# JohnLonginotto/uq

Measured on NVIDIA B200. Metric: fastq_to_uq_encode_reads_per_s, higher is better.
Workload: dtype u8

## Files before the change

### uq_b200/csrc/hist_units.cuh

```cuda
#pragma once
#include "tile.cuh"

#define H2_THREADS 1024
#define H2_QLO 33u
#define H2_ROWS 95
#define H2_COLS 512
#define H2_NOHINT 0x00060402u

struct h2_core {
    unsigned hist_b[256];
    unsigned hist_q[H2_ROWS + 1];
    int state[256];
    unsigned hints, dirty, oor, qmax;
};

__device__ __forceinline__ uint4 lds_v4(uint32_t a) {
    uint4 v;
    asm volatile("ld.shared.v4.u32 {%0, %1, %2, %3}, [%4];" : "=r"(v.x), "=r"(v.y), "=r"(v.z), "=r"(v.w) : "r"(a));
    return v;
}
__device__ __forceinline__ uint32_t h2_unitmask(int lo, int hi) {
    const uint32_t l = lo < 0 ? 0u : (uint32_t)lo, h = hi > 16 ? 16u : (uint32_t)hi;
    return h > l ? (((1u << h) - 1u) & ~((1u << l) - 1u)) : 0u;
}
__device__ __forceinline__ uint32_t h2_nibble_bytes(uint32_t nib) {
    return (((nib & 15u) * 0x00204081u) & 0x01010101u) * 0xFFu;
}

__device__ __forceinline__ unsigned h2_bytesum(unsigned x) {
    const unsigned y = (x & 0x00FF00FFu) + ((x >> 8) & 0x00FF00FFu);
    return (y & 0xFFFFu) + (y >> 16);
}

__device__ __forceinline__ void h2_slow_byte(h2_core* S, unsigned b, unsigned q) {
    atomicAdd(&S->hist_b[b], 1u);
    int f = S->state[b];
    if (f != (int)q && f != 256) {
        if (f < 0) {
            const int old = atomicCAS(&S->state[b], -1, (int)q);
            if (old >= 0 && old != (int)q) { S->state[b] = 256; S->dirty = 1u; }
        } else {
            S->state[b] = 256; S->dirty = 1u;
        }
    }
}

struct h2_dna_acc {
    unsigned p0, p1, p01;
    unsigned ocnt;
    unsigned words, zeroed, noff;
};

__device__ __noinline__ void h2_dna_flush_vals(h2_core* S, unsigned p0, unsigned p1, unsigned p01, unsigned ocnt, unsigned words,
                                               unsigned zeroed, unsigned H) {
    const unsigned s0 = h2_bytesum(p0), s1 = h2_bytesum(p1) >> 1, s01 = h2_bytesum(p01);
    const unsigned n3 = s01, n1 = s0 - s01, n2 = s1 - s01, n0 = 4u * words - zeroed - n1 - n2 - n3;
    const unsigned v0 = n0 - (ocnt & 255u), v1 = n1 - ((ocnt >> 8) & 255u), v2 = n2 - ((ocnt >> 16) & 255u), v3 = n3 - (ocnt >> 24);
    if (v0) atomicAdd(&S->hist_b[H & 255u], v0);
    if (v1) atomicAdd(&S->hist_b[(H >> 8) & 255u], v1);
    if (v2) atomicAdd(&S->hist_b[(H >> 16) & 255u], v2);
    if (v3) atomicAdd(&S->hist_b[H >> 24], v3);
}
__device__ __forceinline__ void h2_dna_flush(h2_core* S, h2_dna_acc& A, unsigned H) {
    h2_dna_flush_vals(S, A.p0, A.p1, A.p01, A.ocnt, A.words, A.zeroed, H);
    A.p0 = A.p1 = A.p01 = A.ocnt = A.words = A.zeroed = A.noff = 0;
}

__device__ __forceinline__ void h2_dna_flush_warp(h2_core* S, h2_dna_acc& A, unsigned H, unsigned lane) {
    unsigned s0 = h2_bytesum(A.p0), s1 = h2_bytesum(A.p1) >> 1, s01 = h2_bytesum(A.p01);
    unsigned nw = A.words, nz = A.zeroed;
    unsigned oc[4];
#pragma unroll
    for (unsigned c = 0; c < 4; c++) oc[c] = (A.ocnt >> (8 * c)) & 255u;
    s0 = __reduce_add_sync(0xffffffffu, s0); s1 = __reduce_add_sync(0xffffffffu, s1); s01 = __reduce_add_sync(0xffffffffu, s01);
    nw = __reduce_add_sync(0xffffffffu, nw); nz = __reduce_add_sync(0xffffffffu, nz);
#pragma unroll
    for (unsigned c = 0; c < 4; c++) oc[c] = __reduce_add_sync(0xffffffffu, oc[c]);
    if (lane == 0 && nw) {
        unsigned n[4];
        n[3] = s01; n[1] = s0 - s01; n[2] = s1 - s01;
        n[0] = 4u * nw - nz - n[1] - n[2] - n[3];
#pragma unroll
        for (unsigned c = 0; c < 4; c++) {
            const unsigned v = n[c] - oc[c];
            if (v) atomicAdd(&S->hist_b[(H >> (8 * c)) & 255u], v);
        }
    }
    A.p0 = A.p1 = A.p01 = A.ocnt = A.words = A.zeroed = A.noff = 0;
}

__device__ __forceinline__ void h2_dna_unit(h2_core* S, const uint4 v, uint32_t ua, uint32_t delta, int lo, int hi, unsigned H,
                                            h2_dna_acc& A) {
    unsigned w[4] = {v.x, v.y, v.z, v.w}, t[4], bad[4];
#pragma unroll
    for (int k = 0; k < 4; k++) {
        t[k] = (w[k] >> 1) & 0x03030303u;
        const unsigned u2 = t[k] | (t[k] >> 4);
        const unsigned sel = __byte_perm(u2, 0u, 0x4420);
        unsigned ex;
        asm("prmt.b32 %0, %1, %2, %3;" : "=r"(ex) : "r"(H), "r"(0u), "r"(sel));
        bad[k] = ex ^ w[k];
    }
    if (lo > 0 || hi < 16) {
        const uint32_t vb = h2_unitmask(lo, hi);
#pragma unroll
        for (int k = 0; k < 4; k++) {
            const unsigned vm = h2_nibble_bytes(vb >> (4 * k));
            bad[k] &= vm;
            t[k] &= vm;
        }
        A.zeroed += 16u - __popc(vb);
    }
    if (bad[0] | bad[1] | bad[2] | bad[3]) {
        unsigned m = 0;
#pragma unroll
        for (int k = 0; k < 4; k++) {
            const unsigned z = (((bad[k] & 0x7F7F7F7Fu) + 0x7F7F7F7Fu) | bad[k]) & 0x80808080u;
            m |= z >> (7 - k);
        }
        A.noff += __popc(m);
        do {
            const unsigned i = (unsigned)__ffs((int)m) - 1u;
            m &= m - 1u;
            const unsigned pos = 4u * (i & 7u) + (i >> 3);
            const unsigned b = lds_u8(ua + pos), q = lds_u8(ua + pos + delta);
            A.ocnt += 1u << (8u * ((b >> 1) & 3u));
            h2_slow_byte(S, b, q);
        } while (m);
    }
#pragma unroll
    for (int k = 0; k < 4; k++) {
        A.p0 += t[k] & 0x01010101u;
        A.p1 += t[k] & 0x02020202u;
        A.p01 += t[k] & (t[k] >> 1) & 0x01010101u;
    }
    A.words += 4u;
}

__device__ __forceinline__ bool h2_qual_unit(const uint4 v, int lo, int hi, uint32_t qcol) {
    unsigned w[4] = {v.x, v.y, v.z, v.w};
    unsigned bad = 0;
    if (lo > 0 || hi < 16) {
        const uint32_t vb = h2_unitmask(lo, hi);
#pragma unroll
        for (int k = 0; k < 4; k++) {
            const unsigned vm = h2_nibble_bytes(vb >> (4 * k));
            const unsigned chk = (w[k] & vm) | (0x21212121u & ~vm);
            bad |= ((chk | (chk + 0x01010101u)) | ~((chk & 0x7F7F7F7Fu) + 0x5F5F5F5Fu)) & 0x80808080u;
            w[k] = (w[k] & vm) | (0x7F7F7F7Fu & ~vm);
        }
    } else {
#pragma unroll
        for (int k = 0; k < 4; k++)
            bad |= ((w[k] | (w[k] + 0x01010101u)) | ~((w[k] & 0x7F7F7F7Fu) + 0x5F5F5F5Fu)) & 0x80808080u;
    }
    if (bad) return false;
#pragma unroll
    for (int k = 0; k < 4; k++) {
#pragma unroll
        for (int j = 0; j < 4; j++) {
            const uint32_t a = qcol + (__byte_perm(w[k], 0u, 0x4440 | j) << 9);
            sts_u8(a, lds_u8m(a) + 1u);
        }
    }
    return true;
}

__device__ __noinline__ void h2_qual_flush(h2_core* S, uint32_t qcol) {
    for (unsigned r = 0; r < H2_ROWS; r++) {
        const uint32_t a = qcol + ((r + H2_QLO) << 9);
        const unsigned c = lds_u8m(a);
        if (c) { atomicAdd(&S->hist_q[r], c); sts_u8(a, 0u); }
    }
}

#define H3_STAGES 3
struct h3_smem {
    alignas(128) uint8_t front_pad[128];
    alignas(128) uint8_t bytes[H3_STAGES][TL_CAP + 32];
    uint32_t loff[H3_STAGES][4 * TL_R + 4];
    alignas(8) uint64_t full[H3_STAGES];
    alignas(8) uint64_t empty[H3_STAGES];
    uint32_t ok[H3_STAGES];
    alignas(16) uint8_t qcnt[H2_ROWS * H2_COLS];
    h2_core C;
};

__device__ __forceinline__ void mbar_arrive(uint64_t* bar) {
    asm volatile("mbarrier.arrive.shared::cta.b64 _, [%0];" ::"r"(smem_u32(bar)) : "memory");
}

__global__ void __launch_bounds__(H2_THREADS, 1) k_pair_hist_pipe(const uint8_t* __restrict__ d, uint64_t n_bytes,
                                                                 const uint64_t* __restrict__ line_off, uint64_t r_begin, uint64_t n_reads,
                                                                 an_dev* __restrict__ s, unsigned int* __restrict__ fallback,
                                                                 uint8_t* __restrict__ names, uint32_t name_pitch) {
    static_assert(TL_R == 128, "thread <-> line binding assumes 128 records per tile");
    extern __shared__ __align__(128) uint8_t h3_raw[];
    h3_smem* S = reinterpret_cast<h3_smem*>(h3_raw);
    const unsigned tid = threadIdx.x, lane = tid & 31u, wid = tid >> 5;
    for (unsigned i = tid; i < H2_ROWS * H2_COLS / 4; i += H2_THREADS) reinterpret_cast<uint32_t*>(S->qcnt)[i] = 0;
    for (unsigned i = tid; i <= H2_ROWS; i += H2_THREADS) S->C.hist_q[i] = 0;
    if (tid < 256) { S->C.hist_b[tid] = 0; S->C.state[tid] = -1; }
    if (tid == 0) {
        S->C.hints = H2_NOHINT; S->C.dirty = 0; S->C.oor = 0; S->C.qmax = 0;
        for (int st = 0; st < H3_STAGES; st++) { mbar_init(&S->full[st], H2_THREADS / 32); mbar_init(&S->empty[st], H2_THREADS / 32); }
        asm volatile("fence.mbarrier_init.release.cluster;" ::: "memory");
    }
    __syncthreads();
    const unsigned line = tid & 255u, rec = line & 127u, k0 = tid >> 8;
    const bool isq = (line >> 7) != 0;
    const bool producer = wid == H2_THREADS / 32 - 1;
    const unsigned cw = ((wid >> 3) << 2) | (wid & 3u);
    const uint32_t qcol = smem_u32(S->qcnt) + lane * 4u + (cw & 3u) + 128u * (cw >> 2) - (H2_QLO << 9);
    unsigned qsym = 0;
    h2_dna_acc A;
    A.p0 = A.p1 = A.p01 = A.ocnt = A.words = A.zeroed = A.noff = 0;
    unsigned H = H2_NOHINT;
    unsigned long long len_min = ~0ull, len_max = 0ull;
    long long bad_plus = LLONG_MAX, bad_len = LLONG_MAX;

    const uint64_t ntiles = (n_reads - r_begin + TL_R - 1) / TL_R;
    const uint32_t K = blockIdx.x < ntiles ? (uint32_t)((ntiles - blockIdx.x + gridDim.x - 1) / gridDim.x) : 0u;

    constexpr uint32_t OPW = (4 * TL_R + 1 + H2_THREADS / 32 - 1) / (H2_THREADS / 32);
    uint64_t pend_off = 0, pend_b0 = 0, pend_b1 = 0;
    const uint64_t rstride = (uint64_t)gridDim.x * TL_R;
    const uint32_t my_off = wid * OPW + lane;
    auto nrec_at = [&](uint64_t r0) { return (uint32_t)(n_reads - r0 < TL_R ? n_reads - r0 : TL_R); };
    auto prep_load = [&](uint64_t r0, uint32_t nrec) {
        const uint64_t* lo = line_off + 4 * r0;
        if (lane < OPW && my_off <= 4 * nrec) pend_off = __ldg(lo + my_off);
        if (producer && lane == 0) { pend_b0 = __ldg(lo); pend_b1 = __ldg(lo + 4 * nrec); }
    };
    auto prep_store = [&](uint32_t nrec, uint32_t st, bool wait_empty, uint32_t empty_par) {
        if (wait_empty) mbar_wait(&S->empty[st], empty_par);
        const uint32_t i = my_off;
        if (lane < OPW && i <= 4 * nrec) S->loff[st][i] = (uint32_t)pend_off;
        if (producer) {
            const uint64_t b0 = __shfl_sync(0xffffffffu, pend_b0, 0), b1 = __shfl_sync(0xffffffffu, pend_b1, 0);
            const uint64_t a0 = b0 & ~15ull;
            const bool fits = b1 - a0 <= TL_CAP;
            uint64_t a1 = (b1 + 15) & ~15ull;
            const uint64_t lim = n_bytes & ~15ull;
            if (a1 > lim) a1 = lim;
            if (a1 < a0) a1 = a0;
            if (fits) for (uint64_t q = a1 + lane; q < b1; q += 32) S->bytes[st][q - a0] = d[q];
            __syncwarp();
            if (lane == 0) {
                S->ok[st] = fits ? 1u : 0u;
                const uint32_t bulk = fits ? (uint32_t)(a1 - a0) : 0u;
                asm volatile("fence.proxy.async.shared::cta;" ::: "memory");
                mbar_expect_tx(&S->full[st], bulk);
                if (bulk) bulk_g2s(S->bytes[st], d + a0, bulk, &S->full[st]);
            }
        } else {
            __syncwarp();
            if (lane == 0) mbar_arrive(&S->full[st]);
        }
    };

    {
        uint64_t r0p = r_begin + (uint64_t)blockIdx.x * TL_R;
        for (uint32_t k = 0; k < K && k < H3_STAGES - 1; k++, r0p += rstride) { const uint32_t nr = nrec_at(r0p); prep_load(r0p, nr); prep_store(nr, k, false, 0u); }
    }
    uint32_t F = 1, next_flush = 1;
    uint64_t r0 = r_begin + (uint64_t)blockIdx.x * TL_R;
    uint32_t st = 0, par = 0;
    for (uint32_t k = 0; k < K; k++) {
        const bool ahead = k + H3_STAGES - 1 < K;
        const uint64_t r0a = r0 + 2 * rstride;
        const uint32_t nrec_a = ahead ? nrec_at(r0a) : 0u;
        const uint32_t st_a = st ? st - 1u : 2u;
        const uint32_t par_a = st ? par : par ^ 1u;
        if (ahead) prep_load(r0a, nrec_a);
        mbar_wait(&S->full[st], par);
        const uint32_t nrec = nrec_at(r0);
        if (S->ok[st] && names && wid < TL_R / 8) {
            const uint32_t bytes_a = smem_u32(S->bytes[st]);
            const uint32_t* loff = S->loff[st];
            const uint32_t base32 = loff[0] & ~15u;
            const uint32_t nr = 8u * wid + (lane >> 2);
            if (nr < nrec) {
                const uint32_t n0 = loff[4 * nr] - base32, nlen = loff[4 * nr + 1] - base32 - n0 - 1u;
                if (nlen + 1u > name_pitch || nlen > 255u) {
                    if ((lane & 3u) == 0) atomicOr(&S->C.oor, 2u);
                } else {
                    uint4* dst = reinterpret_cast<uint4*>(names + (r0 + nr) * name_pitch);
                    for (uint32_t c = lane & 3u; 16u * c <= nlen; c += 4) {
                        const uint32_t at = n0 + 16u * c - 1u, al = bytes_a + (at & ~3u), sh = (at & 3u) * 8u;
                        const uint32_t x0 = lds_u32(al), x1 = lds_u32(al + 4u), x2 = lds_u32(al + 8u), x3 = lds_u32(al + 12u), x4 = lds_u32(al + 16u);
                        uint4 v;
                        v.x = __funnelshift_r(x0, x1, sh); v.y = __funnelshift_r(x1, x2, sh);
                        v.z = __funnelshift_r(x2, x3, sh); v.w = __funnelshift_r(x3, x4, sh);
                        if (c == 0) v.x = (v.x & 0xFFFFFF00u) | nlen;
                        dst[c] = v;
                    }
                }
            }
        }
        if (!S->ok[st]) {
            if (tid == 0) atomicOr(fallback, 1u);
        } else if (rec < nrec) {
            const uint32_t bytes_a = smem_u32(S->bytes[st]);
            const uint32_t* loff = S->loff[st];
            const uint32_t base32 = loff[0] & ~15u;
            const uint32_t o1 = loff[4 * rec + 1] - base32, o2 = loff[4 * rec + 2] - base32, o3 = loff[4 * rec + 3] - base32,
                           o4 = loff[4 * rec + 4] - base32;
            uint32_t len = o2 - o1 - 1;
            const uint32_t qlen = o4 - o3 - 1;
            if (tid < TL_R) {
                const long long r = (long long)(r0 + rec);
                if (len != qlen && r < bad_len) bad_len = r;
                len_min = len < len_min ? len : len_min; len_max = len > len_max ? len : len_max;
                const unsigned plus = o3 - o2 < 2u ? 0u : lds_u8(bytes_a + o2);
                if (plus != '+' && r < bad_plus) bad_plus = r;
            }
            if (qlen < len) len = qlen;
            const uint32_t sb = isq ? o3 : o1, eb = sb + len;
            for (uint32_t u = (sb & ~15u) + 16u * k0; u < eb; u += 64u) {
                const uint4 v = lds_v4(bytes_a + u);
                const int lo = (int)sb - (int)u, hi = (int)eb - (int)u;
                if (isq) {
                    if (qsym > 255u - 16u) { h2_qual_flush(&S->C, qcol); qsym = 0; }
                    if (!h2_qual_unit(v, lo, hi, qcol)) atomicOr(&S->C.oor, 1u);
                    qsym += 16u;
                } else {
                    if (A.words > 120u || A.noff > 224u) h2_dna_flush(&S->C, A, H);
                    h2_dna_unit(&S->C, v, bytes_a + u, o3 - o1, lo, hi, H, A);
                }
            }
        }
        __syncwarp();
        if (lane == 0) mbar_arrive(&S->empty[st]);
        if (ahead) prep_store(nrec_a, st_a, k >= 1, par_a);
        r0 += rstride;
        if (++st == H3_STAGES) { st = 0; par ^= 1u; }
        if (k + 1 == next_flush || k + 1 == K) {
            const unsigned wq = __reduce_max_sync(0xffffffffu, isq ? qsym : 0u);
            if (lane == 0 && wq) atomicMax(&S->C.qmax, wq);
            __syncthreads();
            for (unsigned r = wid; r < H2_ROWS; r += H2_THREADS / 32) {
                uint32_t* row = reinterpret_cast<uint32_t*>(S->qcnt + r * H2_COLS);
                unsigned e = 0, o = 0;
#pragma unroll
                for (int j = 0; j < H2_COLS / 128; j++) {
                    const unsigned x = row[lane + 32 * j];
                    row[lane + 32 * j] = 0;
                    e += x & 0x00FF00FFu; o += (x >> 8) & 0x00FF00FFu;
                }
                unsigned tot = (e & 0xFFFFu) + (e >> 16) + (o & 0xFFFFu) + (o >> 16);
                tot = __reduce_add_sync(0xffffffffu, tot);
                if (lane == 0) S->C.hist_q[r] += tot;
            }
            qsym = 0;
            h2_dna_flush_warp(&S->C, A, H, lane);
            const unsigned m = S->C.qmax;
            __syncthreads();
            if (S->C.dirty && wid == 0) {
                unsigned best[4] = {0, 0, 0, 0};
#pragma unroll
                for (unsigned j = 0; j < 8; j++) {
                    const unsigned b = lane + 32u * j;
                    if (S->C.state[b] == 256) {
                        const unsigned cnt = S->C.hist_b[b] < 0xFFFFFFu ? S->C.hist_b[b] : 0xFFFFFFu;
                        const unsigned key = ((cnt + 1u) << 8) | b;
                        const unsigned c = (b >> 1) & 3u;
#pragma unroll
                        for (unsigned cc = 0; cc < 4; cc++) if (c == cc && key > best[cc]) best[cc] = key;
                    }
                }
                unsigned h = 0;
#pragma unroll
                for (unsigned c = 0; c < 4; c++) {
                    const unsigned mx = __reduce_max_sync(0xffffffffu, best[c]);
                    h |= (mx ? (mx & 255u) : ((H2_NOHINT >> (8 * c)) & 255u)) << (8 * c);
                }
                if (lane == 0) { S->C.hints = h; S->C.dirty = 0; }
            }
            if (tid == 0) S->C.qmax = 0;
            __syncthreads();
            H = S->C.hints;
            const unsigned rate = max(m / F, 16u);
            F = min(max(208u / rate, 1u), 32u);
            next_flush = k + 1 + F;
        }
    }
    if (tid < TL_R) {
#pragma unroll
        for (int o = 16; o > 0; o >>= 1) {
            const unsigned long long a = __shfl_xor_sync(0xffffffffu, len_min, o), b = __shfl_xor_sync(0xffffffffu, len_max, o);
            const long long e = __shfl_xor_sync(0xffffffffu, bad_plus, o), f = __shfl_xor_sync(0xffffffffu, bad_len, o);
            len_min = a < len_min ? a : len_min; len_max = b > len_max ? b : len_max;
            bad_plus = e < bad_plus ? e : bad_plus; bad_len = f < bad_len ? f : bad_len;
        }
        if (lane == 0) {
            if (len_min != ~0ull) atomicMin(&s->dna_min, len_min);
            atomicMax(&s->dna_max, len_max);
            if (bad_plus != LLONG_MAX) atomicMin(&s->bad_plus, bad_plus);
            if (bad_len != LLONG_MAX) atomicMin(&s->bad_len, bad_len);
        }
    }
    __syncthreads();
    if (tid < 256) {
        if (S->C.hist_b[tid]) atomicAdd(&s->base_count[tid], (unsigned long long)S->C.hist_b[tid]);
        if (tid < H2_ROWS - 1 && S->C.hist_q[tid]) atomicAdd(&s->qual_count[tid + H2_QLO], (unsigned long long)S->C.hist_q[tid]);
        if (tid == 0 && (S->C.oor & 1u)) atomicOr(fallback, 1u);
        if (tid == 0 && (S->C.oor & 2u)) atomicOr(fallback, 4u);
        const int f = S->C.state[tid];
        if (f >= 0) {
            if (f == 256) {
                s->multi[tid] = 1;
                atomicCAS(&s->first_q[tid], -1, 0);
            } else {
                const int old = atomicCAS(&s->first_q[tid], -1, f);
                if (old >= 0 && old != f) s->multi[tid] = 1;
            }
        }
    }
}
```

### uq_b200/csrc/split.cu

```cuda
#include "common.cuh"

#define SP_THREADS 256
#define SP_BYTES_PER_THREAD 64
#define SP_TILE (SP_THREADS * SP_BYTES_PER_THREAD)
#define SP_STAGE 1024

__device__ __forceinline__ unsigned nl_bits(unsigned w) {
    const unsigned x = w ^ 0x0A0A0A0Au;
    const unsigned t = ((x & 0x7F7F7F7Fu) + 0x7F7F7F7Fu) | x;
    return (~t & 0x80808080u) >> 7;
}

__device__ __forceinline__ void load_chunk(const uint8_t* __restrict__ d, uint64_t n, uint64_t pos, unsigned (&w)[16]) {
    if (pos + SP_BYTES_PER_THREAD <= n) {
        const uint4* p = reinterpret_cast<const uint4*>(d + pos);
#pragma unroll
        for (int i = 0; i < 4; i++) {
            uint4 q = __ldg(p + i);
            w[4 * i] = q.x; w[4 * i + 1] = q.y; w[4 * i + 2] = q.z; w[4 * i + 3] = q.w;
        }
    } else {
#pragma unroll
        for (int i = 0; i < 16; i++) {
            unsigned x = 0;
#pragma unroll
            for (int b = 0; b < 4; b++) {
                uint64_t q = pos + 4 * i + b;
                if (q < n) x |= (unsigned)d[q] << (8 * b);
            }
            w[i] = x;
        }
    }
}

__global__ void __launch_bounds__(SP_THREADS) k_newline_count(const uint8_t* __restrict__ d, uint64_t n, uint64_t tile0, uint32_t* __restrict__ tile_counts) {
    uint64_t pos = (tile0 + blockIdx.x) * SP_TILE + (uint64_t)threadIdx.x * SP_BYTES_PER_THREAD;
    unsigned c = 0;
    if (pos < n) {
        unsigned w[16];
        load_chunk(d, n, pos, w);
#pragma unroll
        for (int i = 0; i < 16; i++) c += __popc(nl_bits(w[i]));
    }
    __shared__ unsigned ws[SP_THREADS / 32];
#pragma unroll
    for (int o = 16; o > 0; o >>= 1) c += __shfl_xor_sync(0xffffffffu, c, o);
    if (lane_id() == 0) ws[threadIdx.x >> 5] = c;
    __syncthreads();
    if (threadIdx.x == 0) {
        unsigned t = 0;
#pragma unroll
        for (int i = 0; i < SP_THREADS / 32; i++) t += ws[i];
        tile_counts[tile0 + blockIdx.x] = t;
    }
}

__global__ void __launch_bounds__(SP_THREADS) k_newline_write(const uint8_t* __restrict__ d, uint64_t n, uint64_t tile0, uint64_t line_base,
                                                            const uint64_t* __restrict__ tile_base, uint64_t* __restrict__ line_off) {
    uint64_t pos = (tile0 + blockIdx.x) * SP_TILE + (uint64_t)threadIdx.x * SP_BYTES_PER_THREAD;
    unsigned long long nl = 0;
    if (pos < n) {
        unsigned w[16];
        load_chunk(d, n, pos, w);
        unsigned lo = 0, hi = 0;
#pragma unroll
        for (int i = 0; i < 8; i++) {
            lo |= ((nl_bits(w[i]) * 0x01020408u) >> 24) << (4 * i);
            hi |= ((nl_bits(w[8 + i]) * 0x01020408u) >> 24) << (4 * i);
        }
        nl = ((unsigned long long)hi << 32) | lo;
    }
    const unsigned c = __popcll(nl);
    __shared__ unsigned ws[SP_THREADS / 32];
    unsigned lane = lane_id(), wid = threadIdx.x >> 5;
    unsigned incl = c;
#pragma unroll
    for (int o = 1; o < 32; o <<= 1) {
        unsigned t = __shfl_up_sync(0xffffffffu, incl, o);
        if (lane >= (unsigned)o) incl += t;
    }
    if (lane == 31) ws[wid] = incl;
    __syncthreads();
    unsigned wbase = 0;
#pragma unroll
    for (int i = 0; i < SP_THREADS / 32; i++)
        if ((unsigned)i < wid) wbase += ws[i];
    __shared__ uint64_t stage[SP_STAGE];
    __shared__ unsigned tile_total;
    if (threadIdx.x == SP_THREADS - 1) tile_total = wbase + incl;
    __syncthreads();
    const unsigned total = tile_total;
    const uint64_t out0 = line_base + tile_base[tile0 + blockIdx.x] + 1;
    unsigned k = wbase + incl - c;
    const bool staged = total <= SP_STAGE;
    while (nl) {
        const int b = __ffsll((long long)nl) - 1;
        nl &= nl - 1;
        const uint64_t v = pos + b + 1;
        if (staged) stage[k] = v; else line_off[out0 + k] = v;
        k++;
    }
    if (staged) {
        __syncthreads();
        for (unsigned i = threadIdx.x; i < total; i += SP_THREADS) line_off[out0 + i] = stage[i];
    }
}

__global__ void k_set_u64(uint64_t* p, uint64_t v) { *p = v; }

#ifndef SP1_SUB
#define SP1_SUB 4
#endif
struct sp1_smem {
    uint64_t stage[SP_STAGE];
    unsigned ws[SP1_SUB][SP_THREADS / 32];
    unsigned sub_total[SP1_SUB];
    unsigned span;
    unsigned long long prefix;
};

__device__ __forceinline__ unsigned long long sp1_ld(const unsigned long long* p) {
    unsigned long long v;
    asm volatile("ld.volatile.global.u64 %0, [%1];" : "=l"(v) : "l"(p) : "memory");
    return v;
}
__device__ __forceinline__ void sp1_st(unsigned long long* p, unsigned long long v) {
    asm volatile("st.volatile.global.u64 [%0], %1;" ::"l"(p), "l"(v) : "memory");
}

__global__ void __launch_bounds__(SP_THREADS, 8) k_newline_scan1(const uint8_t* __restrict__ d, uint64_t n, uint64_t nspans,
                                                             unsigned int* __restrict__ ticket, unsigned long long* __restrict__ status,
                                                             uint64_t* __restrict__ line_off, uint64_t cap,
                                                             unsigned long long* __restrict__ total_out, unsigned int* __restrict__ overflow) {
    __shared__ sp1_smem S;
    const unsigned tid = threadIdx.x, lane = tid & 31u, wid = tid >> 5;
    const uint64_t span = blockIdx.x;
    (void)ticket;
    if (span >= nspans) return;
    unsigned long long nl[SP1_SUB];
    unsigned incl[SP1_SUB];
#pragma unroll
    for (int q = 0; q < SP1_SUB; q++) {
        const uint64_t pos = (span * SP1_SUB + q) * SP_TILE + (uint64_t)tid * SP_BYTES_PER_THREAD;
        nl[q] = 0;
        if (pos < n) {
            unsigned w[16];
            load_chunk(d, n, pos, w);
            unsigned lo = 0, hi = 0;
#pragma unroll
            for (int i = 0; i < 8; i++) {
                lo |= ((nl_bits(w[i]) * 0x01020408u) >> 24) << (4 * i);
                hi |= ((nl_bits(w[8 + i]) * 0x01020408u) >> 24) << (4 * i);
            }
            nl[q] = ((unsigned long long)hi << 32) | lo;
        }
        unsigned x = __popcll(nl[q]);
#pragma unroll
        for (int o = 1; o < 32; o <<= 1) {
            const unsigned t = __shfl_up_sync(0xffffffffu, x, o);
            if (lane >= (unsigned)o) x += t;
        }
        incl[q] = x;
        if (lane == 31) S.ws[q][wid] = x;
    }
    __syncthreads();
    if (tid < SP1_SUB) {
        unsigned t = 0;
#pragma unroll
        for (int i = 0; i < SP_THREADS / 32; i++) t += S.ws[tid][i];
        S.sub_total[tid] = t;
    }
    __syncthreads();
    unsigned own = 0;
#pragma unroll
    for (int q = 0; q < SP1_SUB; q++) own += S.sub_total[q];
    if (wid == 0) {
        unsigned long long run = 0;
        bool gave_up = false;
        if (span == 0) {
            if (lane == 0) { __threadfence(); sp1_st(status, (2ull << 62) | own); }
        } else {
            if (lane == 0) { __threadfence(); sp1_st(status + span, (1ull << 62) | own); }
            long long at = (long long)span - 1;
            while (true) {
                const long long my = at - (long long)lane;
                unsigned long long v = my >= 0 ? sp1_ld(status + my) : (2ull << 62);
                unsigned spins = 0;
                while (__any_sync(0xffffffffu, (v >> 62) == 0)) {
                    if ((v >> 62) == 0) { __nanosleep(20); v = sp1_ld(status + my); }
                    if ((++spins & 1023u) == 0 && (spins > (1u << 20) || *(volatile unsigned int*)overflow)) { gave_up = true; break; }
                }
                if (gave_up) break;
                const unsigned incl_mask = __ballot_sync(0xffffffffu, (v >> 62) == 2);
                const unsigned upto = incl_mask ? (unsigned)__ffs((int)incl_mask) - 1u : 31u;
                unsigned long long part = lane <= upto ? (v & ((1ull << 62) - 1ull)) : 0ull;
#pragma unroll
                for (int o = 16; o > 0; o >>= 1) part += __shfl_xor_sync(0xffffffffu, part, o);
                run += part;
                if (incl_mask) break;
                at -= 32;
            }
            if (lane == 0 && !gave_up) { __threadfence(); sp1_st(status + span, (2ull << 62) | (run + own)); }
        }
        if (lane == 0) {
            if (gave_up) { atomicOr(overflow, 2u); run = ~0ull >> 2; }
            S.prefix = run;
            if (span == nspans - 1) *total_out = run + own;
        }
    }
    __syncthreads();
    uint64_t out0 = 1 + S.prefix;
    if (out0 + own > cap) {
        if (tid == 0) atomicOr(overflow, 1u);
        return;
    }
#pragma unroll
    for (int q = 0; q < SP1_SUB; q++) {
        const unsigned total = S.sub_total[q];
        if (total) {
            unsigned wbase = 0;
#pragma unroll
            for (int i = 0; i < SP_THREADS / 32; i++)
                if ((unsigned)i < wid) wbase += S.ws[q][i];
            const unsigned c = __popcll(nl[q]);
            unsigned k = wbase + incl[q] - c;
            const bool staged = total <= SP_STAGE;
            const uint64_t pos = (span * SP1_SUB + q) * SP_TILE + (uint64_t)tid * SP_BYTES_PER_THREAD;
            unsigned long long m = nl[q];
            while (m) {
                const int b = __ffsll((long long)m) - 1;
                m &= m - 1;
                const uint64_t v = pos + b + 1;
                if (staged) S.stage[k] = v; else line_off[out0 + k] = v;
                k++;
            }
            if (staged) {
                __syncthreads();
                for (unsigned i = tid; i < total; i += SP_THREADS) line_off[out0 + i] = S.stage[i];
                __syncthreads();
            }
            out0 += total;
        }
    }
}

extern "C" int uqb_fastq_load(uqb_ctx* ctx, const uint8_t* host, uint64_t nbytes, uqb_fastq** out) {
    uqb_fastq* fq = new uqb_fastq();
    uint8_t* d;
    int r = uqb_dalloc(ctx, (void**)&d, nbytes + 64);
    if (r) { delete fq; return r; }
    fq->d = d;
    fq->n = nbytes;
    fq->owned = true;
    UQB_CUDA(cudaMemsetAsync(d + nbytes, 0, 64, ctx->stream));
    if (nbytes) UQB_CUDA(cudaMemcpyAsync(d, host, nbytes, cudaMemcpyHostToDevice, ctx->stream));
    UQB_CUDA(cudaStreamSynchronize(ctx->stream));
    *out = fq;
    return 0;
}

extern "C" int uqb_fastq_adopt(uqb_ctx* ctx, const uint8_t* dev, uint64_t nbytes, uqb_fastq** out) {
    if (((uintptr_t)dev) & 15) return uqb_fail(ctx, "adopted FASTQ buffer must be 16-byte aligned");
    uqb_fastq* fq = new uqb_fastq();
    fq->d = dev;
    fq->n = nbytes;
    fq->owned = false;
    *out = fq;
    return 0;
}

static int free_qcols(uqb_ctx* ctx, uqb_fastq* fq) {
    for (auto& c : fq->qcols) {
        UQB_TRY(uqb_dfree(ctx, c.val, fq->n_reads * 8));
        UQB_TRY(uqb_dfree(ctx, c.span, fq->n_reads * 4));
        UQB_TRY(uqb_dfree(ctx, c.rank, fq->n_reads * 4));
        UQB_TRY(uqb_dfree(ctx, c.first_occ, 0));
        UQB_TRY(uqb_dfree(ctx, c.dict, c.dict_count * c.dict_width + 64));
    }
    fq->qcols.clear();
    return 0;
}

int uqb_fastq_free_qcols(uqb_ctx* ctx, uqb_fastq* fq) { return free_qcols(ctx, fq); }

extern "C" int uqb_fastq_free(uqb_ctx* ctx, uqb_fastq* fq) {
    if (!fq) return 0;
    UQB_TRY(free_qcols(ctx, fq));
    UQB_TRY(uqb_names_release(ctx, fq));
    if (fq->line_off) UQB_TRY(uqb_dfree(ctx, fq->line_off, (fq->n_lines + 1) * 8));
    delete fq->cached_stats;
    if (fq->ref_name) UQB_TRY(uqb_dfree(ctx, fq->ref_name, 0));
    if (fq->owned) UQB_TRY(uqb_dfree(ctx, (void*)fq->d, fq->n + 64));
    delete fq;
    return 0;
}

extern "C" int uqb_fastq_download(uqb_ctx* ctx, const uqb_fastq* fq, uint64_t offset, uint8_t* host, uint64_t nbytes) {
    if (offset + nbytes > fq->n) return uqb_fail(ctx, "fastq download out of range");
    if (nbytes) UQB_CUDA(cudaMemcpyAsync(host, fq->d + offset, nbytes, cudaMemcpyDeviceToHost, ctx->stream));
    UQB_CUDA(cudaStreamSynchronize(ctx->stream));
    return 0;
}

int uqb_split_count_tiles(uqb_ctx* ctx, const uint8_t* d, uint64_t n_end, uint64_t tile0, uint64_t ntiles, uint32_t* counts) {
    UQB_LAUNCH_B(ntiles * SP_TILE, k_newline_count, (unsigned)ntiles, SP_THREADS, 0, d, n_end, tile0, counts);
    return 0;
}
int uqb_split_write_tiles(uqb_ctx* ctx, const uint8_t* d, uint64_t n_end, uint64_t tile0, uint64_t ntiles, uint64_t line_base,
                          const uint64_t* bases, uint64_t* line_off) {
    UQB_LAUNCH_B(ntiles * SP_TILE, k_newline_write, (unsigned)ntiles, SP_THREADS, 0, d, n_end, tile0, line_base, bases, line_off);
    return 0;
}
int uqb_split_set_first(uqb_ctx* ctx, uint64_t* line_off) {
    UQB_LAUNCH(k_set_u64, 1, 1, 0, line_off, 0ull);
    return 0;
}

extern "C" int uqb_split(uqb_ctx* ctx, uqb_fastq* fq, uqb_split_info* info) {
    memset(info, 0, sizeof(*info));
    if (fq->streamed && fq->line_off) {
        info->n_bytes = fq->n; info->n_lines = fq->n_lines; info->n_reads = fq->n_reads;
        info->status = (fq->n_lines % 4 == 0) ? 0 : 1;
        return 0;
    }
    info->n_bytes = fq->n;
    if (fq->line_off) { UQB_TRY(uqb_dfree(ctx, fq->line_off, (fq->n_lines + 1) * 8)); fq->line_off = nullptr; }
    UQB_TRY(uqb_names_release(ctx, fq));
    uint64_t ntiles = (fq->n + SP_TILE - 1) / SP_TILE;
    uint64_t total = 0;
    if (ntiles >= 64) {
        const uint64_t head_tiles = ntiles < 4096 ? ntiles : 4096;
        uint32_t* hc;
        uint64_t *hb, *hd;
        UQB_TRY(uqb_dalloc_t(ctx, &hc, head_tiles));
        UQB_TRY(uqb_dalloc_t(ctx, &hb, head_tiles));
        UQB_TRY(uqb_dalloc_t(ctx, &hd, 1));
        UQB_LAUNCH_B(head_tiles * SP_TILE, k_newline_count, (unsigned)head_tiles, SP_THREADS, 0, fq->d, fq->n, 0ull, hc);
        UQB_TRY(uqb_scan_u32_to_u64(ctx, hc, hb, head_tiles, hd));
        uint64_t head_lines = 0;
        UQB_TRY(uqb_readback(ctx, &head_lines, hd, 8));
        UQB_TRY(uqb_dfree(ctx, hc, 0)); UQB_TRY(uqb_dfree(ctx, hb, 0)); UQB_TRY(uqb_dfree(ctx, hd, 0));
        const double density = (double)head_lines / (double)(head_tiles * SP_TILE);
        const uint64_t cap = (uint64_t)(density * 1.02 * (double)fq->n) + (1u << 20);
        const uint64_t nspans = (ntiles + SP1_SUB - 1) / SP1_SUB;
        uint64_t* lo;
        unsigned long long* status;
        UQB_TRY(uqb_dalloc_t(ctx, &lo, cap + 1));
        UQB_TRY(uqb_dalloc_t(ctx, &status, nspans + 4));
        UQB_CUDA(cudaMemsetAsync(status, 0, (nspans + 4) * 8, ctx->stream));
        UQB_LAUNCH(k_set_u64, 1, 1, 0, lo, 0ull);
        UQB_LAUNCH_B(fq->n + 8 * (uint64_t)(density * (double)fq->n), k_newline_scan1, (unsigned)nspans, SP_THREADS, 0, fq->d, fq->n, nspans,
                     (unsigned int*)(status + nspans), status, lo, cap + 1, status + nspans + 1, (unsigned int*)(status + nspans + 2));
        unsigned long long res[2] = {0, 0};
        UQB_TRY(uqb_readback(ctx, res, status + nspans + 1, 16));
        UQB_TRY(uqb_dfree(ctx, status, 0));
        if ((unsigned int)res[1] == 0) {
            fq->line_off = lo;
            fq->n_lines = res[0];
            fq->n_reads = res[0] / 4;
            info->n_lines = fq->n_lines;
            info->n_reads = fq->n_reads;
            info->status = (fq->n_lines % 4 == 0) ? 0 : 1;
            return 0;
        }
        UQB_TRY(uqb_dfree(ctx, lo, 0));
    }
    uint32_t* counts = nullptr;
    uint64_t* bases = nullptr;
    uint64_t* d_total = nullptr;
    if (ntiles) {
        UQB_TRY(uqb_dalloc_t(ctx, &counts, ntiles));
        UQB_TRY(uqb_dalloc_t(ctx, &bases, ntiles));
        UQB_TRY(uqb_dalloc_t(ctx, &d_total, 1));
        UQB_LAUNCH_B(fq->n, k_newline_count, (unsigned)ntiles, SP_THREADS, 0, fq->d, fq->n, 0ull, counts);
        UQB_TRY(uqb_scan_u32_to_u64(ctx, counts, bases, ntiles, d_total));
        UQB_TRY(uqb_readback(ctx, &total, d_total, 8));
    }
    fq->n_lines = total;
    fq->n_reads = total / 4;
    UQB_TRY(uqb_dalloc_t(ctx, &fq->line_off, total + 1));
    UQB_LAUNCH(k_set_u64, 1, 1, 0, fq->line_off, 0ull);
    if (ntiles) {
        UQB_LAUNCH_B(fq->n + 8 * total, k_newline_write, (unsigned)ntiles, SP_THREADS, 0, fq->d, fq->n, 0ull, 0ull, bases, fq->line_off);
        UQB_TRY(uqb_dfree(ctx, counts, ntiles * 4));
        UQB_TRY(uqb_dfree(ctx, bases, ntiles * 8));
        UQB_TRY(uqb_dfree(ctx, d_total, 8));
    }
    info->n_lines = total;
    info->n_reads = total / 4;
    info->status = (total % 4 == 0) ? 0 : 1;
    return 0;
}

extern "C" int uqb_fastq_line_offsets(uqb_ctx* ctx, const uqb_fastq* fq, uint64_t first, uint64_t count, uint64_t* host) {
    if (!fq->line_off || first + count > fq->n_lines + 1) return uqb_fail(ctx, "line offset range out of bounds");
    if (count) UQB_CUDA(cudaMemcpyAsync(host, fq->line_off + first, count * 8, cudaMemcpyDeviceToHost, ctx->stream));
    UQB_CUDA(cudaStreamSynchronize(ctx->stream));
    return 0;
}
```

### uq_b200/csrc/tile.cuh

```cuda
#pragma once
#include "common.cuh"

#define TL_R 128
#define TL_CAP (48 * 1024)

struct tile_smem {
    alignas(128) uint8_t bytes[TL_CAP + 32];
    uint32_t loff[4 * TL_R + 4];
    alignas(8) uint64_t bar;
};

__device__ __forceinline__ uint32_t smem_u32(const void* p) { return (uint32_t)__cvta_generic_to_shared(p); }

__device__ __forceinline__ uint32_t lds_u8(uint32_t a) {
    uint32_t v;
    asm volatile("ld.shared.u8 %0, [%1];" : "=r"(v) : "r"(a));
    return v;
}
__device__ __forceinline__ uint32_t lds_u32(uint32_t a) {
    uint32_t v;
    asm volatile("ld.shared.u32 %0, [%1];" : "=r"(v) : "r"(a) : "memory");
    return v;
}
__device__ __forceinline__ uint2 lds_u64(uint32_t a) {
    uint2 v;
    asm volatile("ld.shared.v2.u32 {%0, %1}, [%2];" : "=r"(v.x), "=r"(v.y) : "r"(a));
    return v;
}
__device__ __forceinline__ uint32_t lds_u8m(uint32_t a) {
    uint32_t v;
    asm volatile("ld.shared.u8 %0, [%1];" : "=r"(v) : "r"(a) : "memory");
    return v;
}
__device__ __forceinline__ void sts_u8(uint32_t a, uint32_t v) {
    asm volatile("st.shared.u8 [%0], %1;" ::"r"(a), "r"(v) : "memory");
}
__device__ __forceinline__ void sts_u32(uint32_t a, uint32_t v) {
    asm volatile("st.shared.u32 [%0], %1;" ::"r"(a), "r"(v) : "memory");
}

__device__ __forceinline__ void mbar_init(uint64_t* bar, unsigned count) {
    asm volatile("mbarrier.init.shared::cta.b64 [%0], %1;" ::"r"(smem_u32(bar)), "r"(count) : "memory");
}
__device__ __forceinline__ void mbar_expect_tx(uint64_t* bar, unsigned bytes) {
    asm volatile("mbarrier.arrive.expect_tx.shared::cta.b64 _, [%0], %1;" ::"r"(smem_u32(bar)), "r"(bytes) : "memory");
}
__device__ __forceinline__ void bulk_g2s(void* dst, const void* src, unsigned bytes, uint64_t* bar) {
    asm volatile("cp.async.bulk.shared::cluster.global.mbarrier::complete_tx::bytes [%0], [%1], %2, [%3];" ::"r"(smem_u32(dst)),
                 "l"(src), "r"(bytes), "r"(smem_u32(bar))
                 : "memory");
}
__device__ __forceinline__ void mbar_wait(uint64_t* bar, unsigned phase) {
    unsigned ok;
    do {
        asm volatile("{\n .reg .pred p;\n mbarrier.try_wait.parity.shared::cta.b64 p, [%1], %2;\n selp.u32 %0, 1, 0, p;\n}"
                     : "=r"(ok)
                     : "r"(smem_u32(bar)), "r"(phase)
                     : "memory");
    } while (!ok);
}

__device__ __forceinline__ void tile_init(tile_smem* T) {
    if (threadIdx.x == 0) {
        mbar_init(&T->bar, 1);
        asm volatile("fence.mbarrier_init.release.cluster;" ::: "memory");
    }
}

__device__ __forceinline__ uint32_t tile_load(tile_smem* T, const uint8_t* __restrict__ d, uint64_t n_bytes,
                                              const uint64_t* __restrict__ line_off, uint64_t r0, uint64_t r1, unsigned phase,
                                              uint64_t* a0_out) {
    __syncthreads();
    const uint32_t nrec = (uint32_t)(r1 - r0);
    const uint64_t b0 = line_off[4 * r0], b1 = line_off[4 * r1];
    const uint64_t a0 = b0 & ~15ull;
    *a0_out = a0;
    if (b1 - a0 > TL_CAP) return 0;
    uint64_t a1 = (b1 + 15) & ~15ull;
    const uint64_t lim = n_bytes & ~15ull;
    if (a1 > lim) a1 = lim;
    if (a1 < a0) a1 = a0;
    const uint32_t bulk = (uint32_t)(a1 - a0);
    if (threadIdx.x == 0) {
        asm volatile("fence.proxy.async.shared::cta;" ::: "memory");
        mbar_expect_tx(&T->bar, bulk);
        if (bulk) bulk_g2s(T->bytes, d + a0, bulk, &T->bar);
    }
    for (uint32_t i = threadIdx.x; i <= 4 * nrec; i += blockDim.x) T->loff[i] = (uint32_t)(line_off[4 * r0 + i] - a0);
    for (uint64_t q = a1 + threadIdx.x; q < b1; q += blockDim.x) T->bytes[q - a0] = d[q];
    mbar_wait(&T->bar, phase);
    __syncthreads();
    return nrec;
}
```

Measured before the change: 780.5 million.

## Make newline scan persistent with TMA double-buffering and lagged decoupled prefix

Replaces the one-block-per-span newline scan with a persistent grid sized to resident occupancy. Each block streams its spans through a two-stage bulk-copy (cp.async.bulk + mbarrier) pipeline, and it resolves the global prefix with a windowed lookback over the previous G spans, lagged by three iterations so the status wait is overlapped with counting later spans. The intent is to hide global load latency and lookback spin time in a pass that is bound by memory bandwidth. It adds a lot of shared memory and complexity, and it removes the ntiles>=64 threshold so the path always runs. Forward progress now depends on every block being co-resident.

New measurement: 769.9 million, median of 6. -1.4%, worse.

```diff
diff --git a/uq_b200/csrc/hist_units.cuh b/uq_b200/csrc/hist_units.cuh
--- a/uq_b200/csrc/hist_units.cuh
+++ b/uq_b200/csrc/hist_units.cuh
@@ -14,11 +14,6 @@
     unsigned hints, dirty, oor, qmax;
 };
 
-__device__ __forceinline__ uint4 lds_v4(uint32_t a) {
-    uint4 v;
-    asm volatile("ld.shared.v4.u32 {%0, %1, %2, %3}, [%4];" : "=r"(v.x), "=r"(v.y), "=r"(v.z), "=r"(v.w) : "r"(a));
-    return v;
-}
 __device__ __forceinline__ uint32_t h2_unitmask(int lo, int hi) {
     const uint32_t l = lo < 0 ? 0u : (uint32_t)lo, h = hi > 16 ? 16u : (uint32_t)hi;
     return h > l ? (((1u << h) - 1u) & ~((1u << l) - 1u)) : 0u;
diff --git a/uq_b200/csrc/split.cu b/uq_b200/csrc/split.cu
--- a/uq_b200/csrc/split.cu
+++ b/uq_b200/csrc/split.cu
@@ -1,4 +1,5 @@
 #include "common.cuh"
+#include "tile.cuh"
 
 #define SP_THREADS 256
 #define SP_BYTES_PER_THREAD 64
@@ -108,139 +109,165 @@
 
 __global__ void k_set_u64(uint64_t* p, uint64_t v) { *p = v; }
 
-#ifndef SP1_SUB
-#define SP1_SUB 4
-#endif
-struct sp1_smem {
+#define SC_THREADS 512
+#define SC_SPAN (SC_THREADS * SP_BYTES_PER_THREAD)
+#define SC_STAGES 2
+#define SC_LAG 3
+#define SC_COUNTED (1ull << 63)
+struct sc_smem {
+    alignas(128) uint8_t bytes[SC_STAGES][SC_SPAN];
     uint64_t stage[SP_STAGE];
-    unsigned ws[SP1_SUB][SP_THREADS / 32];
-    unsigned sub_total[SP1_SUB];
-    unsigned span;
-    unsigned long long prefix;
+    alignas(8) uint64_t full[SC_STAGES];
+    unsigned ws[2][SC_THREADS / 32];
+    unsigned ww[2][SC_THREADS / 32];
+    unsigned stop[2];
+    unsigned long long mask[SC_LAG + 1][SC_THREADS];
+    unsigned rank[SC_LAG + 1][SC_THREADS];
+    unsigned own[SC_LAG + 1];
 };
 
-__device__ __forceinline__ unsigned long long sp1_ld(const unsigned long long* p) {
+__device__ __forceinline__ unsigned long long sc_ld(const unsigned long long* p) {
     unsigned long long v;
     asm volatile("ld.volatile.global.u64 %0, [%1];" : "=l"(v) : "l"(p) : "memory");
     return v;
 }
-__device__ __forceinline__ void sp1_st(unsigned long long* p, unsigned long long v) {
+__device__ __forceinline__ void sc_st(unsigned long long* p, unsigned long long v) {
     asm volatile("st.volatile.global.u64 [%0], %1;" ::"l"(p), "l"(v) : "memory");
 }
 
-__global__ void __launch_bounds__(SP_THREADS, 8) k_newline_scan1(const uint8_t* __restrict__ d, uint64_t n, uint64_t nspans,
-                                                             unsigned int* __restrict__ ticket, unsigned long long* __restrict__ status,
-                                                             uint64_t* __restrict__ line_off, uint64_t cap,
-                                                             unsigned long long* __restrict__ total_out, unsigned int* __restrict__ overflow) {
-    __shared__ sp1_smem S;
+__device__ __forceinline__ uint32_t sc_bulk_bytes(uint64_t span, uint64_t n) {
+    const uint64_t s0 = span * SC_SPAN, lim = n & ~15ull;
+    const uint64_t s1 = s0 + SC_SPAN < lim ? s0 + SC_SPAN : lim;
+    return s1 > s0 ? (uint32_t)(s1 - s0) : 0u;
+}
+
+__device__ __forceinline__ void sc_issue(sc_smem* S, const uint8_t* __restrict__ d, uint64_t n, uint64_t span, unsigned st) {
+    const uint32_t bulk = sc_bulk_bytes(span, n);
+    mbar_expect_tx(&S->full[st], bulk);
+    if (bulk) bulk_g2s(S->bytes[st], d + span * SC_SPAN, bulk, &S->full[st]);
+}
+
+__global__ void __launch_bounds__(SC_THREADS) k_newline_scan(const uint8_t* __restrict__ d, uint64_t n, uint64_t nspans,
+                                                           unsigned long long* __restrict__ status, uint64_t* __restrict__ line_off, uint64_t cap,
+                                                           unsigned long long* __restrict__ total_out, unsigned int* __restrict__ overflow) {
+    extern __shared__ __align__(128) uint8_t sc_raw[];
+    sc_smem* S = reinterpret_cast<sc_smem*>(sc_raw);
     const unsigned tid = threadIdx.x, lane = tid & 31u, wid = tid >> 5;
-    const uint64_t span = blockIdx.x;
-    (void)ticket;
-    if (span >= nspans) return;
-    unsigned long long nl[SP1_SUB];
-    unsigned incl[SP1_SUB];
-#pragma unroll
-    for (int q = 0; q < SP1_SUB; q++) {
-        const uint64_t pos = (span * SP1_SUB + q) * SP_TILE + (uint64_t)tid * SP_BYTES_PER_THREAD;
-        nl[q] = 0;
-        if (pos < n) {
-            unsigned w[16];
-            load_chunk(d, n, pos, w);
-            unsigned lo = 0, hi = 0;
-#pragma unroll
-            for (int i = 0; i < 8; i++) {
-                lo |= ((nl_bits(w[i]) * 0x01020408u) >> 24) << (4 * i);
-                hi |= ((nl_bits(w[8 + i]) * 0x01020408u) >> 24) << (4 * i);
-            }
-            nl[q] = ((unsigned long long)hi << 32) | lo;
-        }
-        unsigned x = __popcll(nl[q]);
+    const uint64_t G = gridDim.x;
+    const uint64_t K = blockIdx.x < nspans ? (nspans - blockIdx.x + G - 1) / G : 0;
+    if (tid == 0) {
+        S->stop[0] = S->stop[1] = 0;
+        for (int s = 0; s < SC_STAGES; s++) mbar_init(&S->full[s], 1);
+        asm volatile("fence.mbarrier_init.release.cluster;" ::: "memory");
+        for (uint64_t k = 0; k < K && k < SC_STAGES; k++) sc_issue(S, d, n, blockIdx.x + k * G, (unsigned)k);
+    }
+    __syncthreads();
+    unsigned st = 0, par = 0;
+    unsigned slot = 0;
+    unsigned long long base = 0;
+    for (uint64_t k = 0; k < K + SC_LAG; k++) {
+        const bool count = k < K, number = k >= SC_LAG;
+        const uint64_t span = blockIdx.x + k * G, pspan = span - SC_LAG * G;
+        const unsigned buf = (unsigned)k & 1u;
+        const unsigned pslot = slot == SC_LAG ? 0u : slot + 1u;
+        const uint64_t wbeg = pspan >= G ? pspan - G + 1 : 0, wlen = number ? pspan - wbeg : 0;
+        unsigned long long w0 = SC_COUNTED;
+        if (tid < wlen) w0 = sc_ld(status + wbeg + tid);
+        unsigned long long nl = 0;
+        const uint64_t pos = span * SC_SPAN + (uint64_t)tid * SP_BYTES_PER_THREAD;
+        if (count) {
+            const uint64_t a1 = span * SC_SPAN + sc_bulk_bytes(span, n);
+            const uint32_t src = smem_u32(S->bytes[st]) + tid * SP_BYTES_PER_THREAD;
+            mbar_wait(&S->full[st], par);
+            if (pos + SP_BYTES_PER_THREAD <= a1) {
+#pragma unroll
+                for (unsigned j = 0; j < 4; j++) {
+                    const unsigned u = (j + (tid >> 1)) & 3u;
+                    const uint4 v = lds_v4(src + 16u * u);
+                    const unsigned m = ((nl_bits(v.x) * 0x01020408u) >> 24) | (((nl_bits(v.y) * 0x01020408u) >> 24) << 4) |
+                                       (((nl_bits(v.z) * 0x01020408u) >> 24) << 8) | (((nl_bits(v.w) * 0x01020408u) >> 24) << 12);
+                    nl |= (unsigned long long)m << (16u * u);
+                }
+            } else if (pos < n) {
+                for (unsigned b = 0; b < SP_BYTES_PER_THREAD; b++) {
+                    const uint64_t q = pos + b;
+                    const unsigned c = q < a1 ? lds_u8(src + b) : q < n ? d[q] : 0u;
+                    if (c == '\n') nl |= 1ull << b;
+                }
+            }
+        }
+        const unsigned c = __popcll(nl);
+        unsigned incl = c;
 #pragma unroll
         for (int o = 1; o < 32; o <<= 1) {
-            const unsigned t = __shfl_up_sync(0xffffffffu, x, o);
-            if (lane >= (unsigned)o) x += t;
-        }
-        incl[q] = x;
-        if (lane == 31) S.ws[q][wid] = x;
-    }
-    __syncthreads();
-    if (tid < SP1_SUB) {
-        unsigned t = 0;
-#pragma unroll
-        for (int i = 0; i < SP_THREADS / 32; i++) t += S.ws[tid][i];
-        S.sub_total[tid] = t;
-    }
-    __syncthreads();
-    unsigned own = 0;
-#pragma unroll
-    for (int q = 0; q < SP1_SUB; q++) own += S.sub_total[q];
-    if (wid == 0) {
-        unsigned long long run = 0;
-        bool gave_up = false;
-        if (span == 0) {
-            if (lane == 0) { __threadfence(); sp1_st(status, (2ull << 62) | own); }
-        } else {
-            if (lane == 0) { __threadfence(); sp1_st(status + span, (1ull << 62) | own); }
-            long long at = (long long)span - 1;
-            while (true) {
-                const long long my = at - (long long)lane;
-                unsigned long long v = my >= 0 ? sp1_ld(status + my) : (2ull << 62);
-                unsigned spins = 0;
-                while (__any_sync(0xffffffffu, (v >> 62) == 0)) {
-                    if ((v >> 62) == 0) { __nanosleep(20); v = sp1_ld(status + my); }
-                    if ((++spins & 1023u) == 0 && (spins > (1u << 20) || *(volatile unsigned int*)overflow)) { gave_up = true; break; }
-                }
-                if (gave_up) break;
-                const unsigned incl_mask = __ballot_sync(0xffffffffu, (v >> 62) == 2);
-                const unsigned upto = incl_mask ? (unsigned)__ffs((int)incl_mask) - 1u : 31u;
-                unsigned long long part = lane <= upto ? (v & ((1ull << 62) - 1ull)) : 0ull;
-#pragma unroll
-                for (int o = 16; o > 0; o >>= 1) part += __shfl_xor_sync(0xffffffffu, part, o);
-                run += part;
-                if (incl_mask) break;
-                at -= 32;
-            }
-            if (lane == 0 && !gave_up) { __threadfence(); sp1_st(status + span, (2ull << 62) | (run + own)); }
-        }
-        if (lane == 0) {
-            if (gave_up) { atomicOr(overflow, 2u); run = ~0ull >> 2; }
-            S.prefix = run;
-            if (span == nspans - 1) *total_out = run + own;
-        }
-    }
-    __syncthreads();
-    uint64_t out0 = 1 + S.prefix;
-    if (out0 + own > cap) {
-        if (tid == 0) atomicOr(overflow, 1u);
-        return;
-    }
-#pragma unroll
-    for (int q = 0; q < SP1_SUB; q++) {
-        const unsigned total = S.sub_total[q];
-        if (total) {
-            unsigned wbase = 0;
-#pragma unroll
-            for (int i = 0; i < SP_THREADS / 32; i++)
-                if ((unsigned)i < wid) wbase += S.ws[q][i];
-            const unsigned c = __popcll(nl[q]);
-            unsigned k = wbase + incl[q] - c;
-            const bool staged = total <= SP_STAGE;
-            const uint64_t pos = (span * SP1_SUB + q) * SP_TILE + (uint64_t)tid * SP_BYTES_PER_THREAD;
-            unsigned long long m = nl[q];
-            while (m) {
-                const int b = __ffsll((long long)m) - 1;
-                m &= m - 1;
-                const uint64_t v = pos + b + 1;
-                if (staged) S.stage[k] = v; else line_off[out0 + k] = v;
-                k++;
+            const unsigned t = __shfl_up_sync(0xffffffffu, incl, o);
+            if (lane >= (unsigned)o) incl += t;
+        }
+        unsigned wsum = 0;
+        for (uint64_t e = tid; e < wlen; e += SC_THREADS) {
+            unsigned long long v = e == tid ? w0 : sc_ld(status + wbeg + e);
+            for (unsigned spins = 1; !(v & SC_COUNTED); spins++) {
+                if ((spins & 63u) == 0 && (spins > (1u << 20) || *(volatile unsigned int*)overflow)) { S->stop[buf] = 1; break; }
+                __nanosleep(32);
+                v = sc_ld(status + wbeg + e);
+            }
+            wsum += (unsigned)v;
+        }
+#pragma unroll
+        for (int o = 16; o > 0; o >>= 1) wsum += __shfl_xor_sync(0xffffffffu, wsum, o);
+        if (lane == 31) { S->ws[buf][wid] = incl; S->ww[buf][wid] = wsum; }
+        __syncthreads();
+        unsigned own = 0, wbase = 0, win = 0;
+#pragma unroll
+        for (int i = 0; i < SC_THREADS / 32; i++) {
+            const unsigned x = S->ws[buf][i];
+            own += x;
+            if ((unsigned)i < wid) wbase += x;
+            win += S->ww[buf][i];
+        }
+        const bool gave_up = S->stop[buf];
+        if (count) {
+            S->mask[slot][tid] = nl;
+            S->rank[slot][tid] = wbase + incl - c;
+        }
+        if (tid == 0 && count) {
+            S->own[slot] = own;
+            sc_st(status + span, SC_COUNTED | own);
+            if (k + SC_STAGES < K) {
+                asm volatile("fence.proxy.async.shared::cta;" ::: "memory");
+                sc_issue(S, d, n, span + SC_STAGES * G, st);
+            }
+        }
+        if (number) {
+            const unsigned p_own = S->own[pslot];
+            const unsigned long long prefix = base + win;
+            base = prefix + p_own;
+            const bool over = 1 + base > cap;
+            if (gave_up || over) {
+                if (tid == 0) atomicOr(overflow, gave_up ? 2u : 1u);
+                for (uint64_t j = k + 1; j < K && j <= k + SC_STAGES; j++) mbar_wait(&S->full[j % SC_STAGES], (unsigned)(j / SC_STAGES) & 1u);
+                break;
+            }
+            if (tid == 0 && pspan == nspans - 1) *total_out = base;
+            const uint64_t out0 = 1 + prefix;
+            const bool staged = p_own <= SP_STAGE;
+            unsigned long long p_nl = S->mask[pslot][tid];
+            const uint64_t p_pos = pspan * SC_SPAN + (uint64_t)tid * SP_BYTES_PER_THREAD;
+            unsigned r = S->rank[pslot][tid];
+            while (p_nl) {
+                const int b = __ffsll((long long)p_nl) - 1;
+                p_nl &= p_nl - 1;
+                const uint64_t v = p_pos + b + 1;
+                if (staged) S->stage[r] = v; else line_off[out0 + r] = v;
+                r++;
             }
             if (staged) {
                 __syncthreads();
-                for (unsigned i = tid; i < total; i += SP_THREADS) line_off[out0 + i] = S.stage[i];
-                __syncthreads();
-            }
-            out0 += total;
-        }
+                for (unsigned i = tid; i < p_own; i += SC_THREADS) line_off[out0 + i] = S->stage[i];
+            }
+        }
+        slot = pslot;
+        if (++st == SC_STAGES) { st = 0; par ^= 1u; }
     }
 }
 
@@ -328,7 +355,7 @@
     UQB_TRY(uqb_names_release(ctx, fq));
     uint64_t ntiles = (fq->n + SP_TILE - 1) / SP_TILE;
     uint64_t total = 0;
-    if (ntiles >= 64) {
+    if (ntiles) {
         const uint64_t head_tiles = ntiles < 4096 ? ntiles : 4096;
         uint32_t* hc;
         uint64_t *hb, *hd;
@@ -342,17 +369,23 @@
         UQB_TRY(uqb_dfree(ctx, hc, 0)); UQB_TRY(uqb_dfree(ctx, hb, 0)); UQB_TRY(uqb_dfree(ctx, hd, 0));
         const double density = (double)head_lines / (double)(head_tiles * SP_TILE);
         const uint64_t cap = (uint64_t)(density * 1.02 * (double)fq->n) + (1u << 20);
-        const uint64_t nspans = (ntiles + SP1_SUB - 1) / SP1_SUB;
+        const uint64_t nspans = (fq->n + SC_SPAN - 1) / SC_SPAN;
+        int per_sm = 0;
+        UQB_CUDA(cudaFuncSetAttribute(k_newline_scan, cudaFuncAttributeMaxDynamicSharedMemorySize, (int)sizeof(sc_smem)));
+        UQB_CUDA(cudaOccupancyMaxActiveBlocksPerMultiprocessor(&per_sm, k_newline_scan, SC_THREADS, sizeof(sc_smem)));
+        if (per_sm < 1) return uqb_fail(ctx, "k_newline_scan does not fit an SM");
+        const uint64_t resident = (uint64_t)per_sm * ctx->sm_count;
+        const unsigned grid = (unsigned)(nspans < resident ? nspans : resident);
         uint64_t* lo;
         unsigned long long* status;
         UQB_TRY(uqb_dalloc_t(ctx, &lo, cap + 1));
-        UQB_TRY(uqb_dalloc_t(ctx, &status, nspans + 4));
-        UQB_CUDA(cudaMemsetAsync(status, 0, (nspans + 4) * 8, ctx->stream));
+        UQB_TRY(uqb_dalloc_t(ctx, &status, nspans + 2));
+        UQB_CUDA(cudaMemsetAsync(status, 0, (nspans + 2) * 8, ctx->stream));
         UQB_LAUNCH(k_set_u64, 1, 1, 0, lo, 0ull);
-        UQB_LAUNCH_B(fq->n + 8 * (uint64_t)(density * (double)fq->n), k_newline_scan1, (unsigned)nspans, SP_THREADS, 0, fq->d, fq->n, nspans,
-                     (unsigned int*)(status + nspans), status, lo, cap + 1, status + nspans + 1, (unsigned int*)(status + nspans + 2));
+        UQB_LAUNCH_B(fq->n + 8 * (uint64_t)(density * (double)fq->n), k_newline_scan, grid, SC_THREADS, sizeof(sc_smem), fq->d, fq->n, nspans,
+                     status, lo, cap + 1, status + nspans, (unsigned int*)(status + nspans + 1));
         unsigned long long res[2] = {0, 0};
-        UQB_TRY(uqb_readback(ctx, res, status + nspans + 1, 16));
+        UQB_TRY(uqb_readback(ctx, res, status + nspans, 16));
         UQB_TRY(uqb_dfree(ctx, status, 0));
         if ((unsigned int)res[1] == 0) {
             fq->line_off = lo;
diff --git a/uq_b200/csrc/tile.cuh b/uq_b200/csrc/tile.cuh
--- a/uq_b200/csrc/tile.cuh
+++ b/uq_b200/csrc/tile.cuh
@@ -25,6 +25,11 @@
 __device__ __forceinline__ uint2 lds_u64(uint32_t a) {
     uint2 v;
     asm volatile("ld.shared.v2.u32 {%0, %1}, [%2];" : "=r"(v.x), "=r"(v.y) : "r"(a));
+    return v;
+}
+__device__ __forceinline__ uint4 lds_v4(uint32_t a) {
+    uint4 v;
+    asm volatile("ld.shared.v4.u32 {%0, %1, %2, %3}, [%4];" : "=r"(v.x), "=r"(v.y), "=r"(v.z), "=r"(v.w) : "r"(a));
     return v;
 }
 __device__ __forceinline__ uint32_t lds_u8m(uint32_t a) {
```
